# bryanlimy/tf2-cyclegan

Hardware: AMD Instinct MI355X
Metric: images/sec (whole node) horse2zebra 256×256 (higher is better)
Workload: dtype bf16; 1 GPU; model=cyclegan-resnet9-patchgan, global_batch=4, per_gpu_batch=4, image_size=256, parallelism=dp1

## Files before the change

### cyclegan_amd/ops/_hip/conv.hip

```cpp

#include <torch/extension.h>
#include <ATen/cuda/CUDAContext.h>

#include "common.h"

namespace cyg {

constexpr int BM = 128, BN = 64, BK = 64;
constexpr int NTHREADS = 256;
constexpr int LDK = BK + 8;

struct ConvParams {
  const short* __restrict__ x;
  const short* __restrict__ w;
  const short* __restrict__ bias;
  short* __restrict__ y;
  int B, H, W, Cin, OH, OW, Cout, KH, KW;
  int stride, pt, pl;
  int reflect;
  int act;  float slope;
  const float* dq;
  const float* dqb;
  long M, KTOT;
  int mtiles, ntiles;
  float* psum;
  float* psq;
  int tps;
};

DEV int xcd_chunk(int bid, int nb) {
  return (nb % 8 == 0) ? (bid % 8) * (nb / 8) + bid / 8 : bid;
}


template <bool IS_CONVT, bool ALIGNED, int STRIDE>
__global__ __launch_bounds__(NTHREADS) void conv_gemm_kernel(ConvParams p) {
  const int stride = STRIDE ? STRIDE : p.stride;
  __shared__ short As[BM][LDK];
  __shared__ short Bs[BN][LDK];
  __shared__ long rowxb[BM];
  __shared__ long rowyb[BM];
  __shared__ int rowih[BM], rowiw[BM];
  __shared__ char rowok[BM];

  const int tid = threadIdx.x;
  const int lane = tid & 63;
  const int wid = tid >> 6;
  const int bid = xcd_chunk(blockIdx.x, gridDim.x);
  const int mt = bid % p.mtiles, nt = bid / p.mtiles;
  const long m0 = (long)mt * BM;
  const int n0 = nt * BN;

  for (int r = tid; r < BM; r += NTHREADS) {
    long m = m0 + r;
    bool ok = m < p.M;
    long mm = ok ? m : 0;
    int ow = (int)(mm % p.OW);
    int oh = (int)((mm / p.OW) % p.OH);
    int b = (int)(mm / ((long)p.OW * p.OH));
    rowok[r] = ok;
    rowxb[r] = (long)b * p.H * p.W * p.Cin;
    rowyb[r] = ((long)(b * p.OH + oh) * p.OW + ow) * p.Cout;
    if (IS_CONVT) {
      rowih[r] = oh + p.pt;
      rowiw[r] = ow + p.pl;
    } else {
      rowih[r] = oh * stride - p.pt;
      rowiw[r] = ow * stride - p.pl;
    }
  }
  __syncthreads();

  v4f acc[4][2] = {};

  const int wr = wid >> 1, wc = wid & 1;
  const int wm0 = wr * 64, wn0 = wc * 32;
  const int fr = lane & 15;
  const int fg = lane >> 4;

  for (long k0 = 0; k0 < p.KTOT; k0 += BK) {
    if (ALIGNED) {
      #pragma unroll 2
      for (int c = tid; c < BM * (BK / 8); c += NTHREADS) {
        int row = c >> 3;
        int kc = (c & 7) * 8;
        long k = k0 + kc;
        v8s val = {};
        if (k < p.KTOT && rowok[row]) {
          int tap = (int)(k / p.Cin);
          int ci = (int)(k - (long)tap * p.Cin);
          int dkh = tap / p.KW, dkw = tap - (tap / p.KW) * p.KW;
          bool valid = true;
          int ih, iw;
          if (IS_CONVT) {
            int nh = rowih[row] - dkh, nw = rowiw[row] - dkw;
            valid = nh >= 0 && nw >= 0 && (nh % stride) == 0 &&
                    (nw % stride) == 0;
            ih = nh / stride; iw = nw / stride;
            valid = valid && ih < p.H && iw < p.W;
          } else {
            ih = rowih[row] + dkh; iw = rowiw[row] + dkw;
            if (p.reflect) {
              ih = mirror_idx(ih, p.H); iw = mirror_idx(iw, p.W);
            } else {
              valid = ih >= 0 && ih < p.H && iw >= 0 && iw < p.W;
            }
          }
          if (valid)
            val = *(const v8s*)(p.x + rowxb[row] + ((long)ih * p.W + iw) * p.Cin + ci);
        }
        *(v8s*)&As[row][kc] = val;
      }
    } else {
      for (int c = tid; c < BM * BK; c += NTHREADS) {
        int row = c >> 6;
        int kc = c & 63;
        long k = k0 + kc;
        short val = 0;
        if (k < p.KTOT && rowok[row]) {
          int tap = (int)(k / p.Cin);
          int ci = (int)(k - (long)tap * p.Cin);
          int dkh = tap / p.KW, dkw = tap - (tap / p.KW) * p.KW;
          bool valid = true;
          int ih, iw;
          if (IS_CONVT) {
            int nh = rowih[row] - dkh, nw = rowiw[row] - dkw;
            valid = nh >= 0 && nw >= 0 && (nh % stride) == 0 &&
                    (nw % stride) == 0;
            ih = nh / stride; iw = nw / stride;
            valid = valid && ih < p.H && iw < p.W;
          } else {
            ih = rowih[row] + dkh; iw = rowiw[row] + dkw;
            if (p.reflect) {
              ih = mirror_idx(ih, p.H); iw = mirror_idx(iw, p.W);
            } else {
              valid = ih >= 0 && ih < p.H && iw >= 0 && iw < p.W;
            }
          }
          if (valid)
            val = p.x[rowxb[row] + ((long)ih * p.W + iw) * p.Cin + ci];
        }
        As[row][kc] = val;
      }
    }

    if (ALIGNED) {
      #pragma unroll 2
      for (int c = tid; c < BN * (BK / 8); c += NTHREADS) {
        int n = c >> 3;
        int kc = (c & 7) * 8;
        long k = k0 + kc;
        v8s val = {};
        if (n0 + n < p.Cout && k < p.KTOT)
          val = *(const v8s*)(p.w + (long)(n0 + n) * p.KTOT + k);
        *(v8s*)&Bs[n][kc] = val;
      }
    } else {
      for (int c = tid; c < BN * BK; c += NTHREADS) {
        int n = c >> 6;
        int kc = c & 63;
        long k = k0 + kc;
        Bs[n][kc] = (n0 + n < p.Cout && k < p.KTOT)
                        ? p.w[(long)(n0 + n) * p.KTOT + k] : (short)0;
      }
    }
    __syncthreads();

    #pragma unroll
    for (int kk = 0; kk < BK; kk += 32) {
      v8bf a0 = *(const v8bf*)&As[wm0 + 0 * 16 + fr][kk + fg * 8];
      v8bf a1 = *(const v8bf*)&As[wm0 + 1 * 16 + fr][kk + fg * 8];
      v8bf a2 = *(const v8bf*)&As[wm0 + 2 * 16 + fr][kk + fg * 8];
      v8bf a3 = *(const v8bf*)&As[wm0 + 3 * 16 + fr][kk + fg * 8];
      v8bf b0 = *(const v8bf*)&Bs[wn0 + 0 * 16 + fr][kk + fg * 8];
      v8bf b1 = *(const v8bf*)&Bs[wn0 + 1 * 16 + fr][kk + fg * 8];
      acc[0][0] = __builtin_amdgcn_mfma_f32_16x16x32_bf16(a0, b0, acc[0][0], 0, 0, 0);
      acc[0][1] = __builtin_amdgcn_mfma_f32_16x16x32_bf16(a0, b1, acc[0][1], 0, 0, 0);
      acc[1][0] = __builtin_amdgcn_mfma_f32_16x16x32_bf16(a1, b0, acc[1][0], 0, 0, 0);
      acc[1][1] = __builtin_amdgcn_mfma_f32_16x16x32_bf16(a1, b1, acc[1][1], 0, 0, 0);
      acc[2][0] = __builtin_amdgcn_mfma_f32_16x16x32_bf16(a2, b0, acc[2][0], 0, 0, 0);
      acc[2][1] = __builtin_amdgcn_mfma_f32_16x16x32_bf16(a2, b1, acc[2][1], 0, 0, 0);
      acc[3][0] = __builtin_amdgcn_mfma_f32_16x16x32_bf16(a3, b0, acc[3][0], 0, 0, 0);
      acc[3][1] = __builtin_amdgcn_mfma_f32_16x16x32_bf16(a3, b1, acc[3][1], 0, 0, 0);
    }
    __syncthreads();
  }

  #pragma unroll
  for (int nf = 0; nf < 2; ++nf) {
    int n = n0 + wn0 + nf * 16 + fr;
    if (n >= p.Cout) continue;
    float bv = p.bias ? b2f(p.bias[n]) : 0.f;
    #pragma unroll
    for (int mf = 0; mf < 4; ++mf) {
      #pragma unroll
      for (int r = 0; r < 4; ++r) {
        int rl = wm0 + mf * 16 + fg * 4 + r;
        if (!rowok[rl]) continue;
        float v = apply_act(acc[mf][nf][r] + bv, p.act, p.slope);
        p.y[rowyb[rl] + n] = f2b(v);
      }
    }
  }
}


template <int BNT>
struct ConvSmemT {
  long rowyb[BM];
  int rowih[BM], rowiw[BM];
  unsigned rowxb[BM];
  char rowok[BM];
  char _pad[16 - (BM % 16 ? BM % 16 : 16)];
  short A[2][BM * BK];
  short Bt[2][BNT * BK];
};

constexpr int NW = 8;

template <bool IS_CONVT, int STRIDE, int BNT, bool PHASED = false>
__global__ __launch_bounds__(NW * 64) void conv_glds_kernel(ConvParams p) {
  constexpr int NT = NW * 64;
  constexpr int API = 16 / NW;
  constexpr int TBI = BNT / 8;
  constexpr int BPI = TBI >= NW ? TBI / NW : 1;
  constexpr int NF = BNT >= 32 ? 2 : 1;
  constexpr int NWC = BNT / (NF * 16);
  constexpr int NWR = NW / NWC;
  constexpr int MF = (BM / NWR) / 16;
  const int stride = STRIDE ? STRIDE : p.stride;
  extern __shared__ __attribute__((aligned(16))) char smem_raw[];
  auto& sm = *reinterpret_cast<ConvSmemT<BNT>*>(smem_raw);

  const int tid = threadIdx.x;
  const int lane = tid & 63;
  const int w = tid >> 6;
  const int bid = (IS_CONVT && STRIDE == 2)
                      ? blockIdx.x : xcd_chunk(blockIdx.x, gridDim.x);
  const int mt = bid % p.mtiles, nt = bid / p.mtiles;
  const int n0 = nt * BNT;

  static_assert(!PHASED || (IS_CONVT && STRIDE == 2), "PHASED");
  const int tpp = PHASED ? (p.mtiles >> 2) : 0;
  const int phase = PHASED ? mt / tpp : 0;
  const int phh = phase >> 1, phw = phase & 1;
  const int OH2 = p.OH >> 1, OW2 = p.OW >> 1;
  const long m0 = PHASED ? (long)(mt - phase * tpp) * BM : (long)mt * BM;
  const int nvh = PHASED ? ((p.KH - phh + 1) >> 1) : 0;
  const int nvw = PHASED ? ((p.KW - phw + 1) >> 1) : 0;
  const long KEFF = PHASED ? (long)nvh * nvw * p.Cin : p.KTOT;

  for (int r = tid; r < BM; r += NT) {
    if (PHASED) {
      long mp = m0 + r;
      long Mp = (long)p.B * OH2 * OW2;
      bool ok = mp < Mp;
      long mm = ok ? mp : 0;
      int owp = (int)(mm % OW2);
      int ohp = (int)((mm / OW2) % OH2);
      int b = (int)(mm / ((long)OW2 * OH2));
      int i = 2 * ohp + ((phh + p.pt) & 1);
      int j = 2 * owp + ((phw + p.pl) & 1);
      sm.rowok[r] = ok && i < p.OH && j < p.OW;
      sm.rowxb[r] = (unsigned)((long)b * p.H * p.W * p.Cin * 2);
      sm.rowyb[r] = ((long)(b * p.OH + i) * p.OW + j) * p.Cout;
      sm.rowih[r] = (i + p.pt - phh) >> 1;
      sm.rowiw[r] = (j + p.pl - phw) >> 1;
    } else {
      long m = m0 + r;
      bool ok = m < p.M;
      long mm = ok ? m : 0;
      int ow = (int)(mm % p.OW);
      int oh = (int)((mm / p.OW) % p.OH);
      int b = (int)(mm / ((long)p.OW * p.OH));
      sm.rowok[r] = ok;
      sm.rowxb[r] = (unsigned)((long)b * p.H * p.W * p.Cin * 2);
      sm.rowyb[r] = ((long)(b * p.OH + oh) * p.OW + ow) * p.Cout;
      if (IS_CONVT) {
        sm.rowih[r] = oh + p.pt;
        sm.rowiw[r] = ow + p.pl;
      } else {
        sm.rowih[r] = oh * stride - p.pt;
        sm.rowiw[r] = ow * stride - p.pl;
      }
    }
  }
  __syncthreads();

  const int lr = lane >> 3;
  const int klog = ((lane & 7) ^ lr) << 3;
  int aih[API], aiw[API];
  unsigned axb[API];
  bool aok[API];
  #pragma unroll
  for (int j = 0; j < API; ++j) {
    int r = (w * API + j) * 8 + lr;
    aih[j] = sm.rowih[r];
    aiw[j] = sm.rowiw[r];
    axb[j] = sm.rowxb[r];
    aok[j] = sm.rowok[r];
  }
  int bn[BPI];
  #pragma unroll
  for (int j = 0; j < BPI; ++j) bn[j] = (w * BPI + j) * 8 + lr + n0;
  const bool bw_on = w * BPI < TBI;
  static_assert(BNT == 16 || BNT == 64 || BNT == 128, "BNT");

  auto rx = __builtin_amdgcn_make_buffer_rsrc(
      (void*)p.x, 0, (unsigned)((long)p.B * p.H * p.W * p.Cin * 2), 0x00020000);
  auto rw = __builtin_amdgcn_make_buffer_rsrc(
      (void*)p.w, 0, (unsigned)(p.Cout * p.KTOT * 2), 0x00020000);

  const int nk = (int)((KEFF + BK - 1) / BK);
  const bool big_ci = p.Cin >= BK;

  long kcur;
  bool kv;
  int ci, dkh, dkw;
  unsigned avo[API];
  bool avalid[API];
  unsigned bvo[BPI];
  bool bnv[BPI];

  auto recompute_a = [&]() {
    #pragma unroll
    for (int j = 0; j < API; ++j) {
      avalid[j] = false;
      avo[j] = 0xFF000000u;
      if (!aok[j]) continue;
      bool valid = true;
      int ih, iw;
      if (PHASED) {
        ih = aih[j] - dkh; iw = aiw[j] - dkw;
        valid = ih >= 0 && iw >= 0 && ih < p.H && iw < p.W;
      } else if (IS_CONVT) {
        int nh = aih[j] - dkh, nw = aiw[j] - dkw;
        valid = nh >= 0 && nw >= 0 && (nh % stride) == 0 && (nw % stride) == 0;
        ih = nh / stride; iw = nw / stride;
        valid = valid && ih < p.H && iw < p.W;
      } else {
        ih = aih[j] + dkh; iw = aiw[j] + dkw;
        if (p.reflect) {
          ih = mirror_idx(ih, p.H); iw = mirror_idx(iw, p.W);
        } else {
          valid = ih >= 0 && ih < p.H && iw >= 0 && iw < p.W;
        }
      }
      if (valid) {
        avalid[j] = true;
        avo[j] = axb[j] + (unsigned)((((long)ih * p.W + iw) * p.Cin + ci) * 2);
      }
    }
  };

  auto recompute_b = [&]() {
    long kw_idx = kcur;
    if (PHASED)
      kw_idx = ((long)(2 * dkh + phh) * p.KW + (2 * dkw + phw)) * p.Cin + ci;
    #pragma unroll
    for (int j = 0; j < BPI; ++j)
      bvo[j] = (unsigned)(((long)bn[j] * p.KTOT + kw_idx) * 2);
  };

  auto decode_tap = [&]() {
    int tap = (int)(kcur / p.Cin);
    ci = (int)(kcur - (long)tap * p.Cin);
    if (PHASED) {
      dkh = tap / nvw;
      dkw = tap - dkh * nvw;
    } else {
      dkh = tap / p.KW;
      dkw = tap - dkh * p.KW;
    }
  };

  auto init_state = [&]() {
    kcur = klog;
    kv = kcur < KEFF;
    decode_tap();
    recompute_a();
    #pragma unroll
    for (int j = 0; j < BPI; ++j) bnv[j] = bn[j] < p.Cout;
    recompute_b();
  };

  auto advance = [&]() {
    kcur += BK;
    kv = kcur < KEFF;
    if (big_ci) {
      ci += BK;
      if (ci >= p.Cin) {
        ci -= p.Cin;
        if (PHASED) {
          if (++dkw == nvw) { dkw = 0; ++dkh; }
        } else {
          if (++dkw == p.KW) { dkw = 0; ++dkh; }
        }
        recompute_a();
        recompute_b();
      } else {
        #pragma unroll
        for (int j = 0; j < API; ++j) avo[j] += BK * 2;
        #pragma unroll
        for (int j = 0; j < BPI; ++j) bvo[j] += BK * 2;
      }
    } else {
      decode_tap();
      recompute_a();
      recompute_b();
    }
  };

  auto stage = [&](int buf) {
    #pragma unroll
    for (int j = 0; j < API; ++j) {
      unsigned vo = (kv && avalid[j]) ? avo[j] : 0xFF000000u;
      __builtin_amdgcn_raw_ptr_buffer_load_lds(
          rx, (__attribute__((address_space(3))) void*)&sm.A[buf][(w * API + j) * 512],
          16, vo, 0, 0, 0);
    }
    if (bw_on) {
      #pragma unroll
      for (int j = 0; j < BPI; ++j) {
        unsigned vo = (kv && bnv[j]) ? bvo[j] : 0xFF000000u;
        __builtin_amdgcn_raw_ptr_buffer_load_lds(
            rw, (__attribute__((address_space(3))) void*)&sm.Bt[buf][(w * BPI + j) * 512],
            16, vo, 0, 0, 0);
      }
    }
  };

  v4f acc[MF][NF] = {};
  const int wr = w / NWC, wc = w % NWC;
  const int wm0 = wr * (MF * 16), wn0 = wc * (NF * 16);
  const int fr = lane & 15;
  const int fg = lane >> 4;
  const int swz = (fr & 7) << 4;

  init_state();
  stage(0);
  __syncthreads();

  for (int kt = 0; kt < nk; ++kt) {
    if (kt + 1 < nk) {
      advance();
      stage((kt + 1) & 1);
    }
    const char* Ab = (const char*)sm.A[kt & 1];
    const char* Bb = (const char*)sm.Bt[kt & 1];
    #pragma unroll
    for (int kk = 0; kk < BK; kk += 32) {
      const int kbyte = (kk + fg * 8) * 2;
      v8bf a[MF], b[NF];
      #pragma unroll
      for (int mf = 0; mf < MF; ++mf)
        a[mf] = *(const v8bf*)(Ab + ((wm0 + mf * 16 + fr) << 7) + (kbyte ^ swz));
      #pragma unroll
      for (int nf = 0; nf < NF; ++nf)
        b[nf] = *(const v8bf*)(Bb + ((wn0 + nf * 16 + fr) << 7) + (kbyte ^ swz));
      #pragma unroll
      for (int mf = 0; mf < MF; ++mf)
        #pragma unroll
        for (int nf = 0; nf < NF; ++nf)
          acc[mf][nf] = __builtin_amdgcn_mfma_f32_16x16x32_bf16(
              a[mf], b[nf], acc[mf][nf], 0, 0, 0);
    }
    __syncthreads();
  }

  float cs[NF] = {}, cq[NF] = {};
  #pragma unroll
  for (int nf = 0; nf < NF; ++nf) {
    int n = n0 + wn0 + nf * 16 + fr;
    if (n >= p.Cout) continue;
    float bv = p.bias ? b2f(p.bias[n]) : 0.f;
    #pragma unroll
    for (int mf = 0; mf < MF; ++mf) {
      #pragma unroll
      for (int r = 0; r < 4; ++r) {
        int rl = wm0 + mf * 16 + fg * 4 + r;
        if (!sm.rowok[rl]) continue;
        float v = apply_act(acc[mf][nf][r] + bv, p.act, p.slope);
        short hv = f2b(v);
        p.y[sm.rowyb[rl] + n] = hv;
        float fv = b2f(hv);
        cs[nf] += fv;
        cq[nf] += fv * fv;
      }
    }
  }

  if (p.psum != nullptr) {
    float* red = reinterpret_cast<float*>(sm.A[0]);
    static_assert(NWR * BNT * 2 * sizeof(float) <= sizeof(sm.A[0]), "red");
    #pragma unroll
    for (int nf = 0; nf < NF; ++nf) {
      float s = cs[nf], q = cq[nf];
      s += __shfl_xor(s, 16, 64);
      q += __shfl_xor(q, 16, 64);
      s += __shfl_xor(s, 32, 64);
      q += __shfl_xor(q, 32, 64);
      if (fg == 0) {
        int col = wn0 + nf * 16 + fr;
        red[(wr * BNT + col) * 2] = s;
        red[(wr * BNT + col) * 2 + 1] = q;
      }
    }
    __syncthreads();
    if (tid < BNT && n0 + tid < p.Cout) {
      float s = 0.f, q = 0.f;
      #pragma unroll
      for (int k = 0; k < NWR; ++k) {
        s += red[(k * BNT + tid) * 2];
        q += red[(k * BNT + tid) * 2 + 1];
      }
      const int mtl = PHASED ? mt - phase * tpp : mt;
      const int b = mtl / p.tps;
      const int slice = phase * p.tps + (mtl - b * p.tps);
      const long o = ((long)slice * p.B + b) * p.Cout + n0 + tid;
      p.psum[o] = s;
      p.psq[o] = q;
    }
  }
}


constexpr int BKF = 128;
typedef int v4i __attribute__((ext_vector_type(4)));
typedef int v8i __attribute__((ext_vector_type(8)));

struct Fp8Smem {
  unsigned char A[2][BM * BKF];
  unsigned char Bt[2][BN * BKF];
  long rowyb[BM];
  int rowih[BM], rowiw[BM];
  unsigned rowxb[BM];
  char rowok[BM];
};

__global__ void quant_fp8_kernel(const short* __restrict__ x,
                                 const float* __restrict__ scale,
                                 unsigned char* __restrict__ y, long n) {
  long i = ((long)blockIdx.x * blockDim.x + threadIdx.x) * 8;
  float s = scale[0];
  if (i + 8 <= n) {
    v8s v = *(const v8s*)(x + i);
    unsigned char out[8];
    #pragma unroll
    for (int j = 0; j < 8; ++j) {
      out[j] = f2e4m3(b2f(v[j]), s);
    }
    *(uint2*)(y + i) = *(uint2*)out;
  } else if (i < n) {
    for (long k = i; k < n; ++k) {
      y[k] = f2e4m3(b2f(x[k]), scale[0]);
    }
  }
}


__global__ __launch_bounds__(256) void quant_fp8_d_kernel(
    const short* __restrict__ x, const float* __restrict__ amax_prev,
    float* __restrict__ amax_cur, unsigned char* __restrict__ y, long n) {
  const float s = delayed_sx(amax_prev[0]);
  float mx = 0.f;
  long t = (long)blockIdx.x * 256 + threadIdx.x;
  long nthreads = (long)gridDim.x * 256;
  for (long i = t * 8; i + 8 <= n; i += nthreads * 8) {
    v8s v = *(const v8s*)(x + i);
    unsigned char out[8];
    #pragma unroll
    for (int j = 0; j < 8; ++j) {
      float f = b2f(v[j]);
      mx = fmaxf(mx, fabsf(f));
      out[j] = f2e4m3(f, s);
    }
    *(uint2*)(y + i) = *(uint2*)out;
  }
  if (blockIdx.x == 0 && threadIdx.x == 0) {
    for (long k = n & ~7L; k < n; ++k) {
// ... 575 lines not shown
  const long mstart = sl * p.mchunks_per_slice * WG_BM;
  long mend = mstart + p.mchunks_per_slice * WG_BM;
  if (mend > p.M) mend = p.M;
  if (mstart >= mend) {
    long chunk = (((long)sl * p.ktiles + kt) * p.ntiles + nt) *
                 ((long)WBN * WG_BK);
    for (int i = tid; i < WBN * WG_BK; i += NW * 64) p.ws[chunk + i] = 0.f;
    return;
  }

  auto rx = __builtin_amdgcn_make_buffer_rsrc(
      (void*)p.x, 0, (unsigned)((long)p.B * p.H * p.W * p.Cin * 2), 0x00020000);
  auto rd = __builtin_amdgcn_make_buffer_rsrc(
      (void*)p.dy, 0, (unsigned)(p.M * p.Cout * 2), 0x00020000);

  int a_row[API], a_ci[API], a_dkh[API], a_dkw[API];
  bool a_kv[API];
  #pragma unroll
  for (int j = 0; j < API; ++j) {
    int row = (w * API + j) * 4 + (lane >> 4);
    int cb = ((lane & 15) * 16) ^ AXOR(row);
    long k = k0 + cb / 2;
    a_row[j] = row;
    a_kv[j] = k < p.KTOT;
    int tap = a_kv[j] ? (int)(k / p.Cin) : 0;
    a_ci[j] = (int)(k - (long)tap * p.Cin);
    a_dkh[j] = tap / p.KW;
    a_dkw[j] = tap - a_dkh[j] * p.KW;
  }
  const bool dw_on = w * DPI < TDI;
  int d_row[DPI], d_n[DPI];
  #pragma unroll
  for (int j = 0; j < DPI; ++j) {
    int row = (w * DPI + j) * DRPI + lane / DCH;
    int cb = ((lane % DCH) * 16) ^
             (WBN == 128 ? AXOR(row) : WBN == 64 ? DXOR(row) : 0);
    d_row[j] = row;
    d_n[j] = n0 + cb / 2;
  }

  const unsigned C2 = (unsigned)p.Cin * 2;
  const unsigned WC2 = (unsigned)p.W * C2;
  int a_ow[API], a_oh[API], a_b[API], a_ih[API], a_iw[API];
  unsigned avo[API];
  bool ainb[API], avalid[API], a_iw_ok[API];
  unsigned dvo[DPI];

  auto full_a = [&](int j) {
    int ih = a_ih[j], iw = a_iw[j];
    bool valid = a_kv[j];
    if (p.reflect) {
      ih = mirror_idx(ih, p.H); iw = mirror_idx(iw, p.W);
    } else {
      valid = valid && ih >= 0 && ih < p.H && iw >= 0 && iw < p.W;
    }
    avalid[j] = valid;
    avo[j] = valid ? (unsigned)(((((long)a_b[j] * p.H + ih) * p.W + iw) *
                                 p.Cin + a_ci[j]) * 2)
                   : 0xFF000000u;
  };

  #pragma unroll
  for (int j = 0; j < API; ++j) {
    long m = mstart + a_row[j];
    a_ow[j] = (int)(m % p.OW);
    int t = (int)(m / p.OW);
    a_oh[j] = t % p.OH;
    a_b[j] = t / p.OH;
    a_ih[j] = a_oh[j] * p.stride - p.pt + a_dkh[j];
    a_iw[j] = a_ow[j] * p.stride - p.pl + a_dkw[j];
    a_iw_ok[j] = (unsigned)a_iw[j] < (unsigned)p.W;
    ainb[j] = (unsigned)a_ih[j] < (unsigned)p.H && a_iw_ok[j];
    full_a(j);
  }
  #pragma unroll
  for (int j = 0; j < DPI; ++j)
    dvo[j] = d_n[j] < p.Cout
                 ? (unsigned)(((mstart + d_row[j]) * p.Cout + d_n[j]) * 2)
                 : 0xFF000000u;

  const bool ow_fast = (p.OW == WG_BM);
  const unsigned sWC2 = (unsigned)(p.stride * (int)WC2);
  auto advance = [&]() {
    if (ow_fast) {
      #pragma unroll
      for (int j = 0; j < API; ++j) {
        bool rare = (++a_oh[j] >= p.OH);
        if (!rare) {
          int ih = a_ih[j] + p.stride;
          a_ih[j] = ih;
          bool inb = (unsigned)ih < (unsigned)p.H;
          if (inb && ainb[j] && avalid[j]) {
            avo[j] += sWC2;
          } else {
            rare = true;
          }
          ainb[j] = inb && a_iw_ok[j];
        }
        if (rare) {
          while (a_oh[j] >= p.OH) { a_oh[j] -= p.OH; ++a_b[j]; }
          a_ih[j] = a_oh[j] * p.stride - p.pt + a_dkh[j];
          full_a(j);
          ainb[j] = ((unsigned)a_ih[j] < (unsigned)p.H) && a_iw_ok[j];
        }
      }
    } else {
      #pragma unroll
      for (int j = 0; j < API; ++j) {
        int ow0 = a_ow[j], oh0 = a_oh[j], b0 = a_b[j];
        a_ow[j] += WG_BM;
        while (a_ow[j] >= p.OW) { a_ow[j] -= p.OW; ++a_oh[j]; }
        while (a_oh[j] >= p.OH) { a_oh[j] -= p.OH; ++a_b[j]; }
        int dih = (a_oh[j] - oh0) * p.stride;
        int diw = (a_ow[j] - ow0) * p.stride;
        a_ih[j] += dih;
        a_iw[j] += diw;
        bool inb = (unsigned)a_ih[j] < (unsigned)p.H &&
                   (unsigned)a_iw[j] < (unsigned)p.W;
        if (a_b[j] == b0 && inb && ainb[j] && avalid[j]) {
          avo[j] += (unsigned)(dih * (int)WC2 + diw * (int)C2);
        } else {
          full_a(j);
        }
        ainb[j] = inb;
      }
    }
    #pragma unroll
    for (int j = 0; j < DPI; ++j) dvo[j] += (unsigned)(WG_BM * p.Cout * 2);
  };

  auto stage = [&](int buf, long ms, bool tail) {
    #pragma unroll
    for (int j = 0; j < API; ++j) {
      unsigned vo = (!tail || ms + a_row[j] < p.M) ? avo[j] : 0xFF000000u;
      __builtin_amdgcn_raw_ptr_buffer_load_lds(
          rx, (__attribute__((address_space(3))) void*)&sm.A[buf][(w * API + j) * 512],
          16, vo, 0, 0, 0);
    }
    if (dw_on) {
      #pragma unroll
      for (int j = 0; j < DPI; ++j) {
        unsigned vo = (!tail || ms + d_row[j] < p.M) ? dvo[j] : 0xFF000000u;
        __builtin_amdgcn_raw_ptr_buffer_load_lds(
            rd, (__attribute__((address_space(3))) void*)&sm.D[buf][(w * DPI + j) * 512],
            16, vo, 0, 0, 0);
      }
    }
  };

  v4f acc[KF][NFW] = {};
  const int wr = w / NWCW, wc = w % NWCW;
  const int wk0 = wr * (KF * 16), wn0 = wc * (NFW * 16);
  const int fr = lane & 15, fg = lane >> 4;
  const int jg = lane & 15;
  const int tr_row_a = jg >> 2;
  const int tr_cb_a = (jg & 3) * 8;

  int a_base[KF][2], d_base[NFW][2];
  #pragma unroll
  for (int kf = 0; kf < KF; ++kf) {
    #pragma unroll
    for (int h = 0; h < 2; ++h) {
      int row = fg * 8 + tr_row_a + 4 * h;
      int cbl = (wk0 + kf * 16) * 2 + tr_cb_a;
      a_base[kf][h] = row * 256 + (cbl ^ AXOR(row));
    }
  }
  #pragma unroll
  for (int nf = 0; nf < NFW; ++nf) {
    #pragma unroll
    for (int h = 0; h < 2; ++h) {
      int row = fg * 8 + tr_row_a + 4 * h;
      int cbl = (wn0 + nf * 16) * 2 + tr_cb_a;
      d_base[nf][h] = row * (WBN * 2) +
          (cbl ^ (WBN == 128 ? AXOR(row) : WBN == 64 ? DXOR(row) : 0));
    }
  }

  stage(0, mstart, mstart + WG_BM > p.M);
  __syncthreads();

  int cur = 0;
  for (long ms = mstart; ms < mend; ms += WG_BM, cur ^= 1) {
    if (ms + WG_BM < mend) {
      advance();
      stage(cur ^ 1, ms + WG_BM, ms + 2 * WG_BM > p.M);
    }
    const char* Ab = (const char*)sm.A[cur];
    const char* Db = (const char*)sm.D[cur];
    #pragma unroll
    for (int kk = 0; kk < WG_BM; kk += 32) {
      v8bf bfr[NFW];
      #pragma unroll
      for (int nf = 0; nf < NFW; ++nf) {
        v4bfx lo = tr16_read(Db + kk * (WBN * 2) + d_base[nf][0]);
        v4bfx hi = tr16_read(Db + kk * (WBN * 2) + d_base[nf][1]);
        bfr[nf] = __builtin_shufflevector(lo, hi, 0, 1, 2, 3, 4, 5, 6, 7);
      }
      v8bf a[KF];
      #pragma unroll
      for (int kf = 0; kf < KF; ++kf) {
        v4bfx lo = tr16_read(Ab + kk * 256 + a_base[kf][0]);
        v4bfx hi = tr16_read(Ab + kk * 256 + a_base[kf][1]);
        a[kf] = __builtin_shufflevector(lo, hi, 0, 1, 2, 3, 4, 5, 6, 7);
      }
      #pragma unroll
      for (int kf = 0; kf < KF; ++kf)
        #pragma unroll
        for (int nf = 0; nf < NFW; ++nf)
          acc[kf][nf] = __builtin_amdgcn_mfma_f32_16x16x32_bf16(
              a[kf], bfr[nf], acc[kf][nf], 0, 0, 0);
    }
    __syncthreads();
  }

  const long chunk = (((long)sl * p.ktiles + kt) * p.ntiles + nt) *
                     ((long)WBN * WG_BK);
  #pragma unroll
  for (int nf = 0; nf < NFW; ++nf) {
    int nl = wn0 + nf * 16 + fr;
    if (nl >= WBN) continue;
    #pragma unroll
    for (int kf = 0; kf < KF; ++kf) {
      int kl = wk0 + kf * 16 + fg * 4;
      *(float4*)&p.ws[chunk + (long)nl * WG_BK + kl] =
          *(const float4*)&acc[kf][nf];
    }
  }
}

__global__ void wgrad_reduce_kernel(const float* __restrict__ ws,
                                    float* __restrict__ dw, long KTOT,
                                    int Cout, int ktiles, int ntiles,
                                    int slices, int wbn) {
  long idx = (long)blockIdx.x * blockDim.x + threadIdx.x;
  long total = (long)ktiles * WG_BK * ntiles * wbn;
  if (idx >= total) return;
  int kl = (int)(idx % WG_BK);
  long t = idx / WG_BK;
  int kt = (int)(t % ktiles);
  t /= ktiles;
  int nl = (int)(t % wbn);
  int nt = (int)(t / wbn);
  long k = (long)kt * WG_BK + kl;
  int n = nt * wbn + nl;
  if (k >= KTOT || n >= Cout) return;
  long stride = (long)ktiles * ntiles * wbn * WG_BK;
  long off = (((long)kt * ntiles + nt) * wbn + nl) * WG_BK + kl;
  float s0 = 0, s1 = 0, s2 = 0, s3 = 0;
  int sl = 0;
  for (; sl + 4 <= slices; sl += 4) {
    s0 += ws[off + (sl + 0) * stride];
    s1 += ws[off + (sl + 1) * stride];
    s2 += ws[off + (sl + 2) * stride];
    s3 += ws[off + (sl + 3) * stride];
  }
  for (; sl < slices; ++sl) s0 += ws[off + sl * stride];
  dw[(long)n * KTOT + k] = (s0 + s1) + (s2 + s3);
}

__global__ void reflect_fold_kernel(const short* __restrict__ dxp,
                                    short* __restrict__ dx,
                                    int B, int H, int W, int C,
                                    int pt, int pb, int pl, int pr) {
  long idx = (long)blockIdx.x * blockDim.x + threadIdx.x;
  int gpr = C / 8;
  long total = (long)B * H * W * gpr;
  if (idx >= total) return;
  int g = (int)(idx % gpr);
  long t = idx / gpr;
  int j = (int)(t % W);
  t /= W;
  int i = (int)(t % H);
  int b = (int)(t / H);
  int HP = H + pt + pb, WP = W + pl + pr;
  float s[8] = {};
  int hc[3] = {pt + i, pt - i, pt + 2 * (H - 1) - i};
  int wc_[3] = {pl + j, pl - j, pl + 2 * (W - 1) - j};
  #pragma unroll
  for (int a = 0; a < 3; ++a) {
    int qh = hc[a];
    if (qh < 0 || qh >= HP) continue;
    if (a > 0 && qh == hc[0]) continue;
    if (a == 2 && qh == hc[1]) continue;
    if (mirror_idx(qh - pt, H) != i) continue;
    #pragma unroll
    for (int d = 0; d < 3; ++d) {
      int qw = wc_[d];
      if (qw < 0 || qw >= WP) continue;
      if (d > 0 && qw == wc_[0]) continue;
      if (d == 2 && qw == wc_[1]) continue;
      if (mirror_idx(qw - pl, W) != j) continue;
      v8s v = *(const v8s*)(dxp + (((long)b * HP + qh) * WP + qw) * C + g * 8);
      #pragma unroll
      for (int e = 0; e < 8; ++e) s[e] += b2f(v[e]);
    }
  }
  v8s out;
  #pragma unroll
  for (int e = 0; e < 8; ++e) out[e] = f2b(s[e]);
  *(v8s*)(dx + (((long)b * H + i) * W + j) * C + g * 8) = out;
}


static inline int cdiv(long a, long b) { return (int)((a + b - 1) / b); }

template <bool IS_CONVT, bool ALIGNED>
static void launch_conv_s(const ConvParams& p, dim3 grid, hipStream_t stream) {
  switch (p.stride) {
    case 1:
      hipLaunchKernelGGL((conv_gemm_kernel<IS_CONVT, ALIGNED, 1>), grid,
                         dim3(NTHREADS), 0, stream, p);
      break;
    case 2:
      hipLaunchKernelGGL((conv_gemm_kernel<IS_CONVT, ALIGNED, 2>), grid,
                         dim3(NTHREADS), 0, stream, p);
      break;
    default:
      hipLaunchKernelGGL((conv_gemm_kernel<IS_CONVT, ALIGNED, 0>), grid,
                         dim3(NTHREADS), 0, stream, p);
  }
}

static int conv_ntile(int Cout) {
  if (Cout <= 16) return 16;
  return (Cout % 128) == 0 ? 128 : 64;
}

template <bool IS_CONVT, int STRIDE, int BNT, bool PHASED = false>
static void launch_one_glds(const ConvParams& p, hipStream_t stream) {
  constexpr size_t SMB = sizeof(ConvSmemT<BNT>);
  static bool init = []() {
    hipFuncSetAttribute(
        (const void*)(conv_glds_kernel<IS_CONVT, STRIDE, BNT, PHASED>),
        hipFuncAttributeMaxDynamicSharedMemorySize, (int)SMB);
    return true;
  }();
  (void)init;
  hipLaunchKernelGGL((conv_glds_kernel<IS_CONVT, STRIDE, BNT, PHASED>),
                     dim3((long)p.mtiles * p.ntiles), dim3(NW * 64), SMB,
                     stream, p);
  hipError_t err = hipGetLastError();
  TORCH_CHECK(err == hipSuccess, "conv_glds launch failed (BNT=", BNT,
              " PHASED=", PHASED, "): ", hipGetErrorString(err));
}

template <bool IS_CONVT, int BNT>
static void launch_glds_s(const ConvParams& p, hipStream_t stream) {
  switch (p.stride) {
    case 1: launch_one_glds<IS_CONVT, 1, BNT>(p, stream); break;
    case 2: launch_one_glds<IS_CONVT, 2, BNT>(p, stream); break;
    default: launch_one_glds<IS_CONVT, 0, BNT>(p, stream);
  }
}

template <bool IS_CONVT>
static void launch_glds(ConvParams p, hipStream_t stream) {
  const int bnt = conv_ntile(p.Cout);
  p.ntiles = cdiv(p.Cout, bnt);
  switch (bnt) {
    case 16: launch_glds_s<IS_CONVT, 16>(p, stream); break;
    case 128: launch_glds_s<IS_CONVT, 128>(p, stream); break;
    default: launch_glds_s<IS_CONVT, 64>(p, stream);
  }
}

static bool glds_eligible(const ConvParams& p) {
  return (p.Cin % 8) == 0 &&
         (long)p.B * p.H * p.W * p.Cin * 2 < (1L << 31) &&
         (long)p.Cout * p.KTOT * 2 < (1L << 31);
}

static bool phased_eligible(const ConvParams& p, bool is_convt) {
  return glds_eligible(p) && is_convt && p.stride == 2 && (p.OH % 2) == 0 &&
         (p.OW % 2) == 0;
}

static int stats_cap() {
  static const int cap = []() {
    const char* off = getenv("CYG_NO_CONV_STATS");
    if (off && off[0] == '1') return 0;
    const char* e = getenv("CYG_CONV_STATS_MAXSLABS");
    return e ? atoi(e) : 128;
  }();
  return cap;
}

static int stats_slabs(const ConvParams& p, bool is_convt, bool fp8,
                       int* tps) {
  const int cap = stats_cap();
  if (cap <= 0 || p.Cout <= 16 || (p.Cout % 8) != 0) return 0;
  if (!fp8 && !glds_eligible(p)) return 0;
  const bool phased = !fp8 && phased_eligible(p, is_convt);
  const long per = phased ? (long)(p.OH / 2) * (p.OW / 2)
                          : (long)p.OH * p.OW;
  const long ns = (phased ? 4 : 1) * (per / BM);
  if (per % BM != 0 || ns > cap) return 0;
  *tps = (int)(per / BM);
  return (int)ns;
}

static void launch_conv(const ConvParams& p, bool is_convt, hipStream_t stream) {
  if (phased_eligible(p, is_convt)) {
    ConvParams q = p;
    long Mp = (long)q.B * (q.OH / 2) * (q.OW / 2);
    q.mtiles = 4 * cdiv(Mp, BM);
    if (conv_ntile(q.Cout) == 128) {
      q.ntiles = cdiv(q.Cout, 128);
      launch_one_glds<true, 2, 128, true>(q, stream);
    } else {
      launch_one_glds<true, 2, 64, true>(q, stream);
    }
    return;
  }
  if (glds_eligible(p)) {
    if (is_convt) launch_glds<true>(p, stream);
    else launch_glds<false>(p, stream);
    return;
  }
  dim3 grid(p.mtiles * p.ntiles);
  bool aligned = (p.Cin % 8) == 0;
  if (is_convt) {
    if (aligned) launch_conv_s<true, true>(p, grid, stream);
    else launch_conv_s<true, false>(p, grid, stream);
  } else {
    if (aligned) launch_conv_s<false, true>(p, grid, stream);
    else launch_conv_s<false, false>(p, grid, stream);
  }
}

static ConvParams fill_common(const at::Tensor& x, const at::Tensor& w,
                              const c10::optional<at::Tensor>& bias,
                              at::Tensor& y, int stride, int act, double slope) {
  ConvParams p{};
  p.x = (const short*)x.const_data_ptr();
  p.w = (const short*)w.const_data_ptr();
  p.bias = bias.has_value() ? (const short*)bias->const_data_ptr() : nullptr;
  p.y = (short*)y.mutable_data_ptr();
  p.B = x.size(0); p.H = x.size(1); p.W = x.size(2); p.Cin = x.size(3);
  p.OH = y.size(1); p.OW = y.size(2); p.Cout = y.size(3);
  p.KH = w.size(1); p.KW = w.size(2);
  p.stride = stride;
  p.act = act; p.slope = (float)slope;
  p.M = (long)p.B * p.OH * p.OW;
  p.KTOT = (long)p.KH * p.KW * p.Cin;
  p.mtiles = cdiv(p.M, BM);
  p.ntiles = cdiv(p.Cout, BN);
  return p;
}

static void check_conv_inputs(const at::Tensor& x, const at::Tensor& w) {
  TORCH_CHECK(x.is_cuda() && w.is_cuda(), "conv: tensors must be on GPU");
  TORCH_CHECK(x.scalar_type() == at::kBFloat16 && w.scalar_type() == at::kBFloat16,
              "conv: GPU path is bf16 (got ", x.scalar_type(), ")");
  TORCH_CHECK(x.is_contiguous() && w.is_contiguous(), "conv: need contiguous");
  TORCH_CHECK(w.size(3) == x.size(3), "conv: Cin mismatch");
}

static int add_stats(ConvParams& p, bool is_convt, bool fp8, bool want_stats,
                     std::vector<at::Tensor>& out) {
  int tps = 0;
  const int ns = want_stats ? stats_slabs(p, is_convt, fp8, &tps) : 0;
  if (ns > 0) {
    auto ps = at::empty({2, ns, (long)p.B, (long)p.Cout},
                        out[0].options().dtype(at::kFloat));
    p.psum = (float*)ps.mutable_data_ptr();
    p.psq = p.psum + (long)ns * p.B * p.Cout;
    p.tps = tps;
    out.push_back(ps[0]);
    out.push_back(ps[1]);
  }
  return ns;
}

static std::vector<at::Tensor> run_fwd(ConvParams& p, at::Tensor& y,
                                       bool is_convt, bool want_stats) {
  std::vector<at::Tensor> out{y};
  add_stats(p, is_convt, false, want_stats, out);
  launch_conv(p, is_convt, at::cuda::getCurrentCUDAStream());
  return out;
}

static std::vector<at::Tensor> conv2d_fwd_impl(
    at::Tensor x, at::Tensor w, c10::optional<at::Tensor> bias,
    int64_t stride, int64_t pt, int64_t pb, int64_t pl, int64_t pr,
    bool reflect, int64_t act, double slope, bool want_stats) {
  check_conv_inputs(x, w);
  int H = x.size(1), W = x.size(2);
  int KH = w.size(1), KW = w.size(2);
  int OH = (H + pt + pb - KH) / stride + 1;
  int OW = (W + pl + pr - KW) / stride + 1;
  auto y = at::empty({x.size(0), OH, OW, w.size(0)}, x.options());
  auto p = fill_common(x, w, bias, y, stride, act, slope);
  p.pt = pt; p.pl = pl; p.reflect = reflect ? 1 : 0;
  return run_fwd(p, y, false, want_stats);
}

static std::vector<at::Tensor> convt2d_fwd_impl(
    at::Tensor x, at::Tensor w, c10::optional<at::Tensor> bias,
    int64_t stride, int64_t pt, int64_t pl, int64_t out_h, int64_t out_w,
    int64_t act, double slope, bool want_stats) {
  check_conv_inputs(x, w);
  auto y = at::empty({x.size(0), out_h, out_w, w.size(0)}, x.options());
  auto p = fill_common(x, w, bias, y, stride, act, slope);
  p.pt = pt; p.pl = pl; p.reflect = 0;
  return run_fwd(p, y, true, want_stats);
}

at::Tensor conv2d_fwd(at::Tensor x, at::Tensor w, c10::optional<at::Tensor> bias,
                      int64_t stride, int64_t pt, int64_t pb, int64_t pl,
                      int64_t pr, bool reflect, int64_t act, double slope) {
  return conv2d_fwd_impl(x, w, bias, stride, pt, pb, pl, pr, reflect, act,
                         slope, false)[0];
}

std::vector<at::Tensor> conv2d_fwd_stats(
    at::Tensor x, at::Tensor w, c10::optional<at::Tensor> bias,
    int64_t stride, int64_t pt, int64_t pb, int64_t pl, int64_t pr,
    bool reflect, int64_t act, double slope) {
  return conv2d_fwd_impl(x, w, bias, stride, pt, pb, pl, pr, reflect, act,
                         slope, true);
}

at::Tensor convt2d_fwd(at::Tensor x, at::Tensor w, c10::optional<at::Tensor> bias,
                       int64_t stride, int64_t pt, int64_t pl,
                       int64_t out_h, int64_t out_w, int64_t act, double slope) {
  return convt2d_fwd_impl(x, w, bias, stride, pt, pl, out_h, out_w, act,
                          slope, false)[0];
}

std::vector<at::Tensor> convt2d_fwd_stats(
    at::Tensor x, at::Tensor w, c10::optional<at::Tensor> bias,
    int64_t stride, int64_t pt, int64_t pl, int64_t out_h, int64_t out_w,
    int64_t act, double slope) {
  return convt2d_fwd_impl(x, w, bias, stride, pt, pl, out_h, out_w, act,
                          slope, true);
}

at::Tensor conv2d_dgrad(at::Tensor dy, at::Tensor wt, int64_t H, int64_t W,
                        int64_t stride, int64_t pt, int64_t pb, int64_t pl,
                        int64_t pr, bool reflect) {
  check_conv_inputs(dy, wt);
  auto stream = at::cuda::getCurrentCUDAStream();
  if (!reflect) {
    auto dx = at::empty({dy.size(0), H, W, wt.size(0)}, dy.options());
    auto p = fill_common(dy, wt, c10::nullopt, dx, stride, ACT_NONE, 0.0);
    p.pt = pt; p.pl = pl;
    launch_conv(p, true, stream);
    return dx;
  }
  long HP = H + pt + pb, WP = W + pl + pr;
  auto dxp = at::empty({dy.size(0), HP, WP, wt.size(0)}, dy.options());
  auto p = fill_common(dy, wt, c10::nullopt, dxp, stride, ACT_NONE, 0.0);
  p.pt = 0; p.pl = 0;
  launch_conv(p, true, stream);
  auto dx = at::empty({dy.size(0), H, W, wt.size(0)}, dy.options());
  TORCH_CHECK(wt.size(0) % 8 == 0, "reflect dgrad: Cin % 8 != 0");
  long total = dx.numel() / 8;
  int threads = 256;
  hipLaunchKernelGGL(reflect_fold_kernel, dim3(cdiv(total, threads)),
                     dim3(threads), 0, stream,
                     (const short*)dxp.const_data_ptr(),
                     (short*)dx.mutable_data_ptr(),
                     (int)dy.size(0), (int)H, (int)W, (int)wt.size(0),
                     (int)pt, (int)pb, (int)pl, (int)pr);
  return dx;
}

at::Tensor convt2d_dgrad(at::Tensor dy, at::Tensor wt, int64_t IH, int64_t IW,
                         int64_t stride, int64_t pt, int64_t pl) {
  check_conv_inputs(dy, wt);
  int KH = wt.size(1), KW = wt.size(2);
  auto dx = at::empty({dy.size(0), IH, IW, wt.size(0)}, dy.options());
  auto p = fill_common(dy, wt, c10::nullopt, dx, stride, ACT_NONE, 0.0);
  p.pt = pt; p.pl = pl; p.reflect = 0;
  launch_conv(p, false, at::cuda::getCurrentCUDAStream());
  return dx;
}

struct WgSplit { int slices; long mchunks_per_slice; };
static WgSplit wgrad_split(long M, int ktiles, int ntiles) {
  static const int tgt_blocks = []() {
    const char* e = getenv("CYG_WG_BLOCKS");
    return e ? atoi(e) : 512;
  }();
  const long mchunks = (M + WG_BM - 1) / WG_BM;
  const int target = std::max<long>(1, tgt_blocks / ((long)ktiles * ntiles));
  const int slices = (int)std::min<long>(mchunks, target);
  const long per = (mchunks + slices - 1) / slices;
  return {(int)((mchunks + per - 1) / per), per};
}

template <int WBN>
static void launch_wgrad_glds(const WgradParams& p, dim3 grid,
                              hipStream_t stream) {
  constexpr size_t SMB = sizeof(WgSmemT<WBN>);
  if constexpr (WBN == 128) {
    static bool init = []() {
      hipFuncSetAttribute((const void*)(wgrad_glds_kernel<128>),
                          hipFuncAttributeMaxDynamicSharedMemorySize,
                          (int)SMB);
      return true;
    }();
    (void)init;
  }
  hipLaunchKernelGGL((wgrad_glds_kernel<WBN>), grid, dim3(NW * 64), SMB,
                     stream, p);
}

at::Tensor conv2d_wgrad(at::Tensor x, at::Tensor dy, int64_t KH, int64_t KW,
                        int64_t stride, int64_t pt, int64_t pl, bool reflect) {
  TORCH_CHECK(x.is_cuda() && dy.is_cuda() && x.is_contiguous() && dy.is_contiguous());
  TORCH_CHECK(x.scalar_type() == at::kBFloat16 && dy.scalar_type() == at::kBFloat16);
  TORCH_CHECK(dy.size(0) == x.size(0));
  WgradParams p{};
  p.x = (const short*)x.const_data_ptr();
  p.dy = (const short*)dy.const_data_ptr();
  p.B = x.size(0); p.H = x.size(1); p.W = x.size(2); p.Cin = x.size(3);
  p.OH = dy.size(1); p.OW = dy.size(2); p.Cout = dy.size(3);
  p.KH = KH; p.KW = KW; p.stride = stride; p.pt = pt; p.pl = pl;
  p.reflect = reflect ? 1 : 0;
  p.M = (long)p.B * p.OH * p.OW;
  p.KTOT = (long)KH * KW * p.Cin;
  const bool glds_ok = (p.Cin % 8) == 0 && (p.Cout % 8) == 0 &&
                       (long)p.B * p.H * p.W * p.Cin * 2 < (1L << 31) &&
                       p.M * p.Cout * 2 < (1L << 31);
  const int wbn = glds_ok ? conv_ntile(p.Cout) : WG_BN;
  p.ktiles = cdiv(p.KTOT, WG_BK);
  p.ntiles = cdiv(p.Cout, wbn);
  const WgSplit split = wgrad_split(p.M, p.ktiles, p.ntiles);
  p.slices = split.slices;
  p.mchunks_per_slice = split.mchunks_per_slice;
  dim3 grid((long)p.ktiles * p.ntiles * p.slices);
  auto stream = at::cuda::getCurrentCUDAStream();
  if (!glds_ok) {
    auto dw = at::zeros({p.Cout, (long)KH, (long)KW, p.Cin},
                        x.options().dtype(at::kFloat));
    p.dw = (float*)dw.mutable_data_ptr();
    hipLaunchKernelGGL(wgrad_kernel, grid, dim3(NTHREADS), 0, stream, p);
    return dw;
  }
  auto dw = at::empty({p.Cout, (long)KH, (long)KW, p.Cin},
                      x.options().dtype(at::kFloat));
  p.dw = (float*)dw.mutable_data_ptr();
  auto ws = at::empty({(long)p.slices * p.ktiles * p.ntiles * wbn * WG_BK},
                      x.options().dtype(at::kFloat));
  p.ws = (float*)ws.mutable_data_ptr();
  switch (wbn) {
    case 16: launch_wgrad_glds<16>(p, grid, stream); break;
    case 128: launch_wgrad_glds<128>(p, grid, stream); break;
    default: launch_wgrad_glds<64>(p, grid, stream);
  }
  long total = (long)p.ktiles * WG_BK * p.ntiles * wbn;
  hipLaunchKernelGGL(wgrad_reduce_kernel, dim3(cdiv(total, 256)),
                     dim3(256), 0, stream,
                     (const float*)ws.const_data_ptr(), p.dw, p.KTOT,
                     p.Cout, p.ktiles, p.ntiles, p.slices, wbn);
  return dw;
}

at::Tensor quant_fp8(at::Tensor x, at::Tensor scale) {
  TORCH_CHECK(x.is_cuda() && x.scalar_type() == at::kBFloat16 && x.is_contiguous());
  TORCH_CHECK(scale.scalar_type() == at::kFloat);
  auto y = at::empty_like(x, x.options().dtype(at::kByte));
  long n = x.numel();
  long blocks = (n / 8 + 255) / 256 + 1;
  hipLaunchKernelGGL(quant_fp8_kernel, dim3((unsigned)blocks), dim3(256), 0,
                     at::cuda::getCurrentCUDAStream(),
                     (const short*)x.const_data_ptr(),
                     (const float*)scale.const_data_ptr(),
                     (unsigned char*)y.mutable_data_ptr(), n);
  return y;
}

at::Tensor quant_fp8_d(at::Tensor x, at::Tensor amax_prev,
                       at::Tensor amax_cur) {
  TORCH_CHECK(x.is_cuda() && x.scalar_type() == at::kBFloat16 &&
              x.is_contiguous());
  TORCH_CHECK(amax_prev.scalar_type() == at::kFloat &&
              amax_cur.scalar_type() == at::kFloat);
  auto y = at::empty_like(x, x.options().dtype(at::kByte));
  long n = x.numel();
  long blocks = std::min<long>((n / 8 + 255) / 256 + 1, 768);
  hipLaunchKernelGGL(quant_fp8_d_kernel, dim3((unsigned)blocks), dim3(256), 0,
                     at::cuda::getCurrentCUDAStream(),
                     (const short*)x.const_data_ptr(),
                     (const float*)amax_prev.const_data_ptr(),
                     (float*)amax_cur.mutable_data_ptr(),
                     (unsigned char*)y.mutable_data_ptr(), n);
  return y;
}

void amax_roll(at::Tensor arena, int64_t n) {
  TORCH_CHECK(arena.is_cuda() && arena.scalar_type() == at::kFloat &&
              arena.dim() == 2 && arena.size(0) == 2 && arena.is_contiguous());
  int cap = (int)arena.size(1);
  TORCH_CHECK(n <= cap);
  hipLaunchKernelGGL(amax_roll_kernel, dim3(cdiv(n, 256)), dim3(256), 0,
                     at::cuda::getCurrentCUDAStream(),
                     (float*)arena.mutable_data_ptr(), (int)n, cap);
}

static std::vector<at::Tensor> conv2d_fp8_fwd_impl(
    at::Tensor xq, at::Tensor wq, at::Tensor dq, c10::optional<at::Tensor> sw,
    c10::optional<at::Tensor> bias, int64_t stride, int64_t pt, int64_t pb,
    int64_t pl, int64_t pr, bool reflect, int64_t act, double slope,
    bool want_stats) {
  TORCH_CHECK(xq.is_cuda() && xq.scalar_type() == at::kByte && xq.is_contiguous());
  TORCH_CHECK(wq.scalar_type() == at::kByte && wq.is_contiguous());
  TORCH_CHECK(xq.size(3) == wq.size(3) && xq.size(3) % 16 == 0,
              "fp8 conv: Cin % 16 != 0");
  int H = xq.size(1), W = xq.size(2);
  int KH = wq.size(1), KW = wq.size(2);
  int OH = (H + pt + pb - KH) / stride + 1;
  int OW = (W + pl + pr - KW) / stride + 1;
  auto y = at::empty({xq.size(0), OH, OW, wq.size(0)},
                     xq.options().dtype(at::kBFloat16));
  auto p = fill_common(xq, wq, bias, y, stride, act, slope);
  p.pt = pt; p.pl = pl; p.reflect = reflect ? 1 : 0;
  p.dq = (const float*)dq.const_data_ptr();
  p.dqb = sw.has_value() ? (const float*)sw->const_data_ptr() : nullptr;
  TORCH_CHECK((long)p.B * H * W * p.Cin < (1L << 31) &&
              (long)p.Cout * p.KTOT < (1L << 31));
  std::vector<at::Tensor> out{y};
  const int ns = add_stats(p, false, true, want_stats, out);
  auto stream = at::cuda::getCurrentCUDAStream();
  dim3 grid(p.mtiles * p.ntiles);
#define LAUNCH_FP8(S)                                                        \
  do {                                                                       \
    if (ns > 0)                                                              \
      hipLaunchKernelGGL((conv_fp8_kernel<S, true>), grid, dim3(NTHREADS),   \
                         0, stream, p);                                      \
    else                                                                     \
      hipLaunchKernelGGL((conv_fp8_kernel<S, false>), grid, dim3(NTHREADS),  \
                         0, stream, p);                                      \
  } while (0)
  switch (p.stride) {
    case 1: LAUNCH_FP8(1); break;
    case 2: LAUNCH_FP8(2); break;
    default: LAUNCH_FP8(0);
  }
#undef LAUNCH_FP8
  return out;
}

at::Tensor conv2d_fp8_fwd(at::Tensor xq, at::Tensor wq, at::Tensor dq,
                          c10::optional<at::Tensor> sw,
                          c10::optional<at::Tensor> bias, int64_t stride,
                          int64_t pt, int64_t pb, int64_t pl, int64_t pr,
                          bool reflect, int64_t act, double slope) {
  return conv2d_fp8_fwd_impl(xq, wq, dq, sw, bias, stride, pt, pb, pl, pr,
                             reflect, act, slope, false)[0];
}

std::vector<at::Tensor> conv2d_fp8_fwd_stats(
    at::Tensor xq, at::Tensor wq, at::Tensor dq, c10::optional<at::Tensor> sw,
    c10::optional<at::Tensor> bias, int64_t stride, int64_t pt, int64_t pb,
    int64_t pl, int64_t pr, bool reflect, int64_t act, double slope) {
  return conv2d_fp8_fwd_impl(xq, wq, dq, sw, bias, stride, pt, pb, pl, pr,
                             reflect, act, slope, true);
}

}
```

Before: 335.2 images/s.

## Write reflect-pad dgrad interior directly to dx and fold only border ring

For stride-1 reflect-padded conv backward-data, the transposed-conv GEMM now writes interior pixels straight into the final dx layout and sends padding-ring pixels to a separate ring buffer. A small kernel then adds the mirrored ring contributions into the border pixels of dx only. This replaces the full padded-tensor fold pass, which read and rewrote every pixel, and removes one full-size allocation and copy. It adds per-row index math in the GEMM prologue and extra complexity in the ring indexing.

```diff
diff --git a/cyclegan_amd/ops/_hip/conv.hip b/cyclegan_amd/ops/_hip/conv.hip
--- a/cyclegan_amd/ops/_hip/conv.hip
+++ b/cyclegan_amd/ops/_hip/conv.hip
@@ -26,7 +26,16 @@
   float* psum;
   float* psq;
   int tps;
+  long ringoff;
+  int wt, wl, wH, wW;
 };
+
+DEV int ring_index(int qh, int qw, int OH, int OW, int wt, int wl, int wH,
+                   int wW) {
+  if (qh < wt) return qh * OW + qw;
+  if (qh >= wt + wH) return (qh - wH) * OW + qw;
+  return (OH - wH) * OW + (qh - wt) * (OW - wW) + (qw < wl ? qw : qw - wW);
+}
 
 DEV int xcd_chunk(int bid, int nb) {
   return (nb % 8 == 0) ? (bid % 8) * (nb / 8) + bid / 8 : bid;
@@ -275,7 +284,19 @@
       int b = (int)(mm / ((long)p.OW * p.OH));
       sm.rowok[r] = ok;
       sm.rowxb[r] = (unsigned)((long)b * p.H * p.W * p.Cin * 2);
-      sm.rowyb[r] = ((long)(b * p.OH + oh) * p.OW + ow) * p.Cout;
+      long yb = ((long)(b * p.OH + oh) * p.OW + ow) * p.Cout;
+      if (IS_CONVT && p.ringoff != 0) {
+        const int i = oh - p.wt, j = ow - p.wl;
+        if ((unsigned)i < (unsigned)p.wH && (unsigned)j < (unsigned)p.wW) {
+          yb = (((long)b * p.wH + i) * p.wW + j) * p.Cout;
+        } else {
+          const long rp = (long)p.OH * p.OW - (long)p.wH * p.wW;
+          yb = p.ringoff +
+               (b * rp + ring_index(oh, ow, p.OH, p.OW, p.wt, p.wl, p.wH,
+                                    p.wW)) * p.Cout;
+        }
+      }
+      sm.rowyb[r] = yb;
       if (IS_CONVT) {
         sm.rowih[r] = oh + p.pt;
         sm.rowiw[r] = ow + p.pl;
@@ -1457,8 +1478,92 @@
   *(v8s*)(dx + (((long)b * H + i) * W + j) * C + g * 8) = out;
 }
 
+struct Span2 { int a0, n0, a1, n1; };
+DEV int span_nth(Span2 s, int k) {
+  return k < s.n0 ? s.a0 + k : s.a1 + (k - s.n0);
+}
+DEV int span_nth_out(Span2 s, int k) {
+  if (k >= s.a0) k += s.n0;
+  if (k >= s.a1) k += s.n1;
+  return k;
+}
+
+__global__ void reflect_ring_add_kernel(short* __restrict__ dx,
+                                        const short* __restrict__ ring,
+                                        int B, int H, int W, int C,
+                                        int pt, int pb, int pl, int pr,
+                                        Span2 rs, Span2 cs) {
+  long idx = (long)blockIdx.x * blockDim.x + threadIdx.x;
+  const int gpr = C / 8;
+  const int nr = rs.n0 + rs.n1, nc = cs.n0 + cs.n1;
+  const int ppb = nr * W + (H - nr) * nc;
+  long total = (long)B * ppb * gpr;
+  if (idx >= total) return;
+  int g = (int)(idx % gpr);
+  long t = idx / gpr;
+  int q = (int)(t % ppb);
+  int b = (int)(t / ppb);
+  int i, j;
+  if (q < nr * W) {
+    i = span_nth(rs, q / W);
+    j = q % W;
+  } else {
+    q -= nr * W;
+    i = span_nth_out(rs, q / nc);
+    j = span_nth(cs, q % nc);
+  }
+  int HP = H + pt + pb, WP = W + pl + pr;
+  long rp = (long)HP * WP - (long)H * W;
+  short* own = dx + (((long)b * H + i) * W + j) * C + g * 8;
+  float s[8] = {};
+  int hc[3] = {pt + i, pt - i, pt + 2 * (H - 1) - i};
+  int wc_[3] = {pl + j, pl - j, pl + 2 * (W - 1) - j};
+  #pragma unroll
+  for (int a = 0; a < 3; ++a) {
+    int qh = hc[a];
+    if (qh < 0 || qh >= HP) continue;
+    if (a > 0 && qh == hc[0]) continue;
+    if (a == 2 && qh == hc[1]) continue;
+    if (mirror_idx(qh - pt, H) != i) continue;
+    #pragma unroll
+    for (int d = 0; d < 3; ++d) {
+      int qw = wc_[d];
+      if (qw < 0 || qw >= WP) continue;
+      if (d > 0 && qw == wc_[0]) continue;
+      if (d == 2 && qw == wc_[1]) continue;
+      if (mirror_idx(qw - pl, W) != j) continue;
+      const short* src = (a == 0 && d == 0)
+          ? own
+          : ring + (b * rp + ring_index(qh, qw, HP, WP, pt, pl, H, W)) * C +
+                g * 8;
+      v8s v = *(const v8s*)src;
+      #pragma unroll
+      for (int e = 0; e < 8; ++e) s[e] += b2f(v[e]);
+    }
+  }
+  v8s out;
+  #pragma unroll
+  for (int e = 0; e < 8; ++e) out[e] = f2b(s[e]);
+  *(v8s*)own = out;
+}
+
 
 static inline int cdiv(long a, long b) { return (int)((a + b - 1) / b); }
+
+static inline bool env_flag(const char* v) { return v && v[0] == '1'; }
+
+static Span2 mirror_span(int n, int lo, int hi) {
+  const int a0 = 1, b0 = std::min(lo, n - 1);
+  const int a1 = std::max(n - 1 - hi, 0), b1 = n - 2;
+  const int n0 = std::max(b0 - a0 + 1, 0), n1 = std::max(b1 - a1 + 1, 0);
+  if (n0 == 0) return {a1, n1, a1 + n1, 0};
+  if (n1 == 0) return {a0, n0, a0 + n0, 0};
+  if (a1 <= a0 + n0) {
+    const int a = std::min(a0, a1), b = std::max(b0, b1);
+    return {a, b - a + 1, b + 1, 0};
+  }
+  return {a0, n0, a1, n1};
+}
 
 template <bool IS_CONVT, bool ALIGNED>
 static void launch_conv_s(const ConvParams& p, dim3 grid, hipStream_t stream) {
@@ -1704,15 +1809,33 @@
     launch_conv(p, true, stream);
     return dx;
   }
+  TORCH_CHECK(wt.size(0) % 8 == 0, "reflect dgrad: Cin % 8 != 0");
   long HP = H + pt + pb, WP = W + pl + pr;
-  auto dxp = at::empty({dy.size(0), HP, WP, wt.size(0)}, dy.options());
+  const long B = dy.size(0), C = wt.size(0);
+  const long nimg = B * H * W * C;
+  auto dxp = at::empty({B, HP, WP, C}, dy.options());
   auto p = fill_common(dy, wt, c10::nullopt, dxp, stride, ACT_NONE, 0.0);
   p.pt = 0; p.pl = 0;
+  int threads = 256;
+  if (stride == 1 && HP * WP > H * W && glds_eligible(p) &&
+      !env_flag(getenv("CYG_NO_DIRECT_FOLD"))) {
+    auto dx = dxp.view({-1}).narrow(0, 0, nimg).view({B, H, W, C});
+    p.ringoff = nimg;
+    p.wt = pt; p.wl = pl; p.wH = H; p.wW = W;
+    launch_conv(p, true, stream);
+    const Span2 rs = mirror_span(H, pt, pb), cs = mirror_span(W, pl, pr);
+    const long nr = rs.n0 + rs.n1, nc = cs.n0 + cs.n1;
+    const long total = B * (nr * W + (H - nr) * nc) * (C / 8);
+    if (total > 0)
+      hipLaunchKernelGGL(reflect_ring_add_kernel, dim3(cdiv(total, threads)),
+                         dim3(threads), 0, stream, p.y, p.y + nimg, (int)B,
+                         (int)H, (int)W, (int)C, (int)pt, (int)pb, (int)pl,
+                         (int)pr, rs, cs);
+    return dx;
+  }
   launch_conv(p, true, stream);
-  auto dx = at::empty({dy.size(0), H, W, wt.size(0)}, dy.options());
-  TORCH_CHECK(wt.size(0) % 8 == 0, "reflect dgrad: Cin % 8 != 0");
+  auto dx = at::empty({B, H, W, C}, dy.options());
   long total = dx.numel() / 8;
-  int threads = 256;
   hipLaunchKernelGGL(reflect_fold_kernel, dim3(cdiv(total, threads)),
                      dim3(threads), 0, stream,
                      (const short*)dxp.const_data_ptr(),
```

Result: faster. 340.1 images/s (median of 6 runs) (+1.4%).
